# hippylib/hippyflow

Measured on AMD Instinct MI355X. Metric: randomized-SVD throughput (GDoF*rank/s), higher is better.
Workload: dtype f64

## Files before the change

hippyflow_amd/csrc/hfmi_gemm.hip:

```cpp
#include "hfmi_gemm_common.h"

#ifdef HFMI_TN_NT
#define TN_LOAD_A(p) __builtin_nontemporal_load(p)
#else
#define TN_LOAD_A(p) (*(p))
#endif
struct TnTail {
  int nrb, nsplit;
  int64_t chunk;
  double* out;
  int64_t si, sj, sps;
};

template <int MT, int NT, bool TR, int WAVES, int R4>
__global__ __launch_bounds__(WAVES * 64, (WAVES == 8 || MT * NT <= 20) ? 2 : 1) void k_tsgemm_tn(const double* __restrict__ A, int64_t lda, int m,
                                                                    const double* B , int64_t ldb, int k,
                                                                    int64_t Npad, int64_t chunk, int nrb, int nsplit,
                                                                    double* __restrict__ out, int64_t si, int64_t sj,
                                                                    int64_t sps, int direct, int probe_arg, TnTail tail) {
#ifdef HFMI_TN_PROBE
  const int probe = probe_arg;
#else
  constexpr int probe = 0;
  (void)probe_arg;
#endif
  extern __shared__ __attribute__((aligned(16))) char smem[];
  constexpr int BK = TN_BK;
  constexpr int COLS = NT * 16;
  constexpr int LDB = BK + 2;
  constexpr int BUFD = COLS * LDB;
  constexpr int CSH = 4;
  constexpr int NTF = R4 > 0 ? NT - 1 : NT;
  constexpr int NR4 = R4 > 0 ? R4 : 1;
  constexpr int NTHR = WAVES * 64;
  constexpr int CH = COLS * (BK / 2);
  constexpr int NQ = (CH + NTHR - 1) / NTHR;
  constexpr int EST = MT * NTF * 8 + MT * R4 * 2 + NTF * 4 + R4 * 4 + 16 * MT + NQ * 6;
  constexpr int AH = (EST <= ((WAVES == 8 || MT * NT <= 20) ? 218 : 470)) ? 2 : 1;
  double* lds = reinterpret_cast<double*>(smem);
  const int tid = threadIdx.x, lane = tid & 63, wave = tid >> 6;
  const int r16 = lane & 15, kk = lane >> 4;

  const int nfull = nrb * nsplit;
  const bool in_tail = (int)blockIdx.x >= nfull;
  const int logical = in_tail ? xcd_remap((int)blockIdx.x - nfull, tail.nrb * tail.nsplit) : xcd_remap(blockIdx.x, nfull);
  const int sp = in_tail ? logical / tail.nrb : logical / nrb;
  const int rb = in_tail ? nrb + logical % tail.nrb : logical % nrb;
  if (in_tail) {
    chunk = tail.chunk;
    out = tail.out;
    si = tail.si;
    sj = tail.sj;
    sps = tail.sps;
    direct = 0;
  }
  const int row_off = in_tail ? nrb * (16 * MT * WAVES) : 0;
  const int64_t t_begin = (int64_t)sp * chunk;
  int64_t t_end = t_begin + chunk;
  if (t_end > Npad) t_end = Npad;
  const int nstages = (int)((t_end - t_begin) / BK);
  const int64_t t_last = t_end - 8 * AH;
  const int rowbase = rb * (16 * MT * WAVES) + wave * (16 * MT);

  const double* a_ptr[MT];
#pragma unroll
  for (int mt = 0; mt < MT; ++mt) {
    int row = rowbase + mt * 16 + r16;
    if (row > m - 1) row = m - 1;
    a_ptr[mt] = A + (int64_t)row * lda + kk * 2 * AH;
  }
  const double* b_ptr[NQ];
#pragma unroll
  for (int qd = 0; qd < NQ; ++qd) {
    int c = tid + NTHR * qd;
    if (c > CH - 1) c = CH - 1;
    int col = c >> CSH;
    if (col > k - 1) col = k - 1;
    b_ptr[qd] = B + (int64_t)col * ldb + (c & ((1 << CSH) - 1)) * 2;
  }

  constexpr int NTA = NTF > 0 ? NTF : 1;
  d4 acc[MT][NTA];
  double acc4[MT][NR4];
#pragma unroll
  for (int mt = 0; mt < MT; ++mt) {
#pragma unroll
    for (int nt = 0; nt < NTA; ++nt) acc[mt][nt] = d4{0.0, 0.0, 0.0, 0.0};
#pragma unroll
    for (int q = 0; q < NR4; ++q) acc4[mt][q] = 0.0;
  }

  d2 breg[NQ];
  auto stage_load = [&](int64_t ts) {
#pragma unroll
    for (int qd = 0; qd < NQ; ++qd) breg[qd] = *reinterpret_cast<const d2*>(b_ptr[qd] + ts);
  };
  auto stage_store = [&](double* L) {
#pragma unroll
    for (int qd = 0; qd < NQ; ++qd) {
      const int c = tid + NTHR * qd;
      const int col = c >> CSH, q = c & ((1 << CSH) - 1);
      const int off = col * LDB + q * 2;
      if (CH % NTHR == 0 || c < CH) *reinterpret_cast<d2*>(L + off) = breg[qd];
    }
  };
  auto load_a = [&](d2(&dst)[AH][MT], int64_t t) {
    if (t > t_last) t = t_last;
    if (probe & 1) t = t_begin;
#pragma unroll
    for (int mt = 0; mt < MT; ++mt)
#pragma unroll
      for (int h = 0; h < AH; ++h) dst[h][mt] = TN_LOAD_A(reinterpret_cast<const d2*>(a_ptr[mt] + t + 2 * h));
  };
  d2 bf[NTA];
  auto koff = [&](int it) { return (it / AH) * (8 * AH) + kk * (2 * AH) + (it % AH) * 2; };
  auto ldsb1 = [&](const double* L, int it, int nt) {
    bf[nt] = *reinterpret_cast<const d2*>(L + (nt * 16 + r16) * LDB + koff(it));
  };
  auto mma = [&](const d2(&a)[MT], const double* L, int it, bool refill) {
    d2 bg[NR4];
    if constexpr (R4 > 0) {
#pragma unroll
      for (int q = 0; q < R4; ++q)
        bg[q] = *reinterpret_cast<const d2*>(L + (NTF * 16 + 4 * q + (lane & 3)) * LDB + koff(it));
    }
#pragma unroll
    for (int nt = 0; nt < NTF; ++nt) {
#pragma unroll
      for (int mt = 0; mt < MT; ++mt)
        acc[mt][nt] = TR ? MFMA_F64(bf[nt].x, a[mt].x, acc[mt][nt]) : MFMA_F64(a[mt].x, bf[nt].x, acc[mt][nt]);
#pragma unroll
      for (int mt = 0; mt < MT; ++mt)
        acc[mt][nt] = TR ? MFMA_F64(bf[nt].y, a[mt].y, acc[mt][nt]) : MFMA_F64(a[mt].y, bf[nt].y, acc[mt][nt]);
      if (refill) ldsb1(L, it + 1, nt);
      __builtin_amdgcn_sched_barrier(0);
    }
    if constexpr (R4 > 0) {
#pragma unroll
      for (int mt = 0; mt < MT; ++mt)
#pragma unroll
        for (int q = 0; q < R4; ++q) acc4[mt][q] = MFMA_F64_4(a[mt].x, bg[q].x, acc4[mt][q]);
#pragma unroll
      for (int mt = 0; mt < MT; ++mt)
#pragma unroll
        for (int q = 0; q < R4; ++q) acc4[mt][q] = MFMA_F64_4(a[mt].y, bg[q].y, acc4[mt][q]);
    }
    __builtin_amdgcn_sched_barrier(0);
  };

  if (nstages > 0) {
    stage_load(t_begin);
    stage_store(lds);
    __syncthreads();
  }
  {
    constexpr int NIT = BK / (8 * AH), NH = BK / 8;
    d2 a[2][AH][MT];
    load_a(a[0], t_begin);
    for (int s = 0; s < nstages; ++s) {
      const int64_t ts = t_begin + (int64_t)s * BK;
      const bool has_next = s + 1 < nstages;
      stage_load(has_next ? ts + BK : ts);
      asm volatile("" ::: "memory");
      const double* L = lds + (s & 1) * BUFD;
#pragma unroll
      for (int nt = 0; nt < NTF; ++nt) ldsb1(L, 0, nt);
#pragma unroll
      for (int it = 0; it < NIT; ++it) {
        load_a(a[(it + 1) & 1], ts + 8 * AH * (it + 1));
#pragma unroll
        for (int h = 0; h < AH; ++h) mma(a[it & 1][h], L, it * AH + h, it * AH + h + 1 < NH);
      }
      if (!(probe & 2)) {
      if (has_next) stage_store(lds + ((s + 1) & 1) * BUFD);
      __syncthreads();
      }
    }
  }

  double* P = out + (int64_t)sp * sps;
#pragma unroll
  for (int mt = 0; mt < MT; ++mt)
#pragma unroll
    for (int nt = 0; nt < NTF; ++nt)
#pragma unroll
      for (int r = 0; r < 4; ++r) {
        const int i = TR ? rowbase + mt * 16 + r16 : rowbase + mt * 16 + kk + 4 * r;
        const int j = TR ? nt * 16 + kk + 4 * r : nt * 16 + r16;
        if (!direct || (i < m && j < k)) P[(int64_t)(i - row_off) * si + (int64_t)j * sj] = acc[mt][nt][r];
      }
  if constexpr (R4 > 0) {
    const int i4 = lane >> 4, g4 = (lane >> 2) & 3, j4 = lane & 3;
#pragma unroll
    for (int mt = 0; mt < MT; ++mt)
#pragma unroll
      for (int q = 0; q < R4; ++q) {
        const int i = rowbase + mt * 16 + 4 * g4 + i4;
        const int j = NTF * 16 + 4 * q + j4;
        if (!direct || (i < m && j < k)) P[(int64_t)(i - row_off) * si + (int64_t)j * sj] = acc4[mt][q];
      }
  }
}

template <int RY>
__global__ __launch_bounds__(64 * RY) void k_reduce_partials(const double* __restrict__ part, int nsplit, int64_t pstride,
                                                             int inner_ld, int tr, int m, int k, double scale, double beta,
                                                             double* __restrict__ C, int64_t rs, int64_t cs) {
  __shared__ double sh[RY][64];
  const int tx = threadIdx.x, ty = threadIdx.y;
  const int fast = blockIdx.x * 64 + tx;
  const int fastn = tr ? m : k, slown = tr ? k : m;
  for (int slow = blockIdx.y; slow < slown; slow += gridDim.y) {
    double s0 = 0.0, s1 = 0.0, s2 = 0.0, s3 = 0.0;
    if (fast < fastn) {
      const double* p = part + (int64_t)slow * inner_ld + fast;
      int sp = ty;
      for (; sp + 3 * RY < nsplit; sp += 4 * RY) {
        s0 += p[(int64_t)sp * pstride];
        s1 += p[(int64_t)(sp + RY) * pstride];
        s2 += p[(int64_t)(sp + 2 * RY) * pstride];
        s3 += p[(int64_t)(sp + 3 * RY) * pstride];
      }
      for (; sp < nsplit; sp += RY) s0 += p[(int64_t)sp * pstride];
    }
    sh[ty][tx] = (s0 + s1) + (s2 + s3);
    __syncthreads();
    if (ty == 0 && fast < fastn) {
      double s = 0.0;
#pragma unroll
      for (int y = 0; y < RY; ++y) s += sh[y][tx];
      const int i = tr ? fast : slow, j = tr ? slow : fast;
      double* out = C + (int64_t)i * rs + (int64_t)j * cs;
      *out = (beta != 0.0) ? scale * s + beta * (*out) : scale * s;
    }
    __syncthreads();
  }
}

template <int RY>
__global__ __launch_bounds__(64 * RY) void k_reduce_flat(const double* __restrict__ part, int nsplit, int64_t pstride,
                                                         int64_t total, int kpad, int k, double scale, double beta,
                                                         double* __restrict__ C) {
  __shared__ double sh[RY][64];
  const int tx = threadIdx.x, ty = threadIdx.y;
  const int64_t idx = (int64_t)blockIdx.x * 64 + tx;
  double s0 = 0.0, s1 = 0.0, s2 = 0.0, s3 = 0.0;
  if (idx < total) {
    const double* p = part + idx;
    int sp = ty;
    for (; sp + 3 * RY < nsplit; sp += 4 * RY) {
      s0 += p[(int64_t)sp * pstride];
      s1 += p[(int64_t)(sp + RY) * pstride];
      s2 += p[(int64_t)(sp + 2 * RY) * pstride];
      s3 += p[(int64_t)(sp + 3 * RY) * pstride];
    }
    for (; sp < nsplit; sp += RY) s0 += p[(int64_t)sp * pstride];
  }
  sh[ty][tx] = (s0 + s1) + (s2 + s3);
  __syncthreads();
  if (ty == 0 && idx < total) {
    double s = 0.0;
#pragma unroll
    for (int y = 0; y < RY; ++y) s += sh[y][tx];
    const bool real = (int)(idx % kpad) < k;
    C[idx] = real ? ((beta != 0.0) ? scale * s + beta * C[idx] : scale * s) : 0.0;
  }
}

__global__ __launch_bounds__(256) void k_reduce_vec(const double* __restrict__ part, int nsplit, int64_t pstride, int64_t prow,
                                                    int64_t rowlen, int nrows, int64_t kpad, int kreal, double scale, double beta,
                                                    double* __restrict__ C, int64_t crow) {
  const int64_t f = ((int64_t)blockIdx.x * 256 + threadIdx.x) * 2;
  if (f >= rowlen) return;
  for (int row = blockIdx.y; row < nrows; row += gridDim.y) {
    const double* p = part + (int64_t)row * prow + f;
    d2 s0 = d2{0.0, 0.0}, s1 = s0, s2 = s0, s3 = s0;
    int sp = 0;
    for (; sp + 3 < nsplit; sp += 4) {
      s0 += *reinterpret_cast<const d2*>(p + (int64_t)sp * pstride);
      s1 += *reinterpret_cast<const d2*>(p + (int64_t)(sp + 1) * pstride);
      s2 += *reinterpret_cast<const d2*>(p + (int64_t)(sp + 2) * pstride);
      s3 += *reinterpret_cast<const d2*>(p + (int64_t)(sp + 3) * pstride);
    }
    for (; sp < nsplit; ++sp) s0 += *reinterpret_cast<const d2*>(p + (int64_t)sp * pstride);
    d2 v = ((s0 + s1) + (s2 + s3)) * scale;
    double* out = C + (int64_t)row * crow + f;
    if (beta != 0.0) v += beta * *reinterpret_cast<const d2*>(out);
    if (kreal < kpad) {
      if ((int)(f % kpad) >= kreal) v.x = 0.0;
      if ((int)((f + 1) % kpad) >= kreal) v.y = 0.0;
    }
    *reinterpret_cast<d2*>(out) = v;
  }
}

int launch_reduce_partials(hfmi_ctx* ctx, const double* part, const reduce_call& c, double scale, double beta, double* C, int64_t rs,
                           int64_t cs) {
  const reduce_plan p = reduce_plan_make(c, rs, cs, (((uintptr_t)part | (uintptr_t)C) & 15) == 0);
  const dim3 grid(p.gx, p.gy);
  switch (p.route) {
    case HFMI_REDUCE_VEC_LONG:
    case HFMI_REDUCE_VEC_ROWS:
      hipLaunchKernelGGL(k_reduce_vec, grid, dim3(256), 0, ctx->stream, part, p.nsplit, c.pstride, (int64_t)c.inner_ld, p.rowlen, p.nrows,
                         p.kpad, p.kreal, scale, beta, C, p.crow);
      break;
    case HFMI_REDUCE_FLAT:
      hipLaunchKernelGGL(p.ry == 4 ? k_reduce_flat<4> : k_reduce_flat<16>, grid, dim3(64, p.ry), 0, ctx->stream, part, p.nsplit, c.pstride,
                         p.rowlen, c.inner_ld, p.k, scale, beta, C);
      break;
    default:
      hipLaunchKernelGGL(p.ry == 4 ? k_reduce_partials<4> : k_reduce_partials<16>, grid, dim3(64, p.ry), 0, ctx->stream, part, p.nsplit,
                         c.pstride, c.inner_ld, p.tr, p.m, p.k, scale, beta, C, rs, cs);
  }
  HIP_TRY(hipGetLastError());
  reduce_plan_words(p, plan_slot(ctx));
  return HFMI_OK;
}

typedef void (*tn_kernel_t)(const double*, int64_t, int, const double*, int64_t, int, int64_t, int64_t, int, int, double*, int64_t, int64_t,
                            int64_t, int, int, TnTail);
template <int MT, int NT, int WAVES>
static tn_kernel_t tn_kernel_r4(bool tr, int r4) {
#define TN_R4(R) \
  case R:        \
    return tr ? k_tsgemm_tn<MT, NT, true, WAVES, R> : k_tsgemm_tn<MT, NT, false, WAVES, R>;
  if constexpr (WAVES == 8) {
    switch (r4) { TN_R4(1) TN_R4(2) TN_R4(3) }
  }
  switch (0) { TN_R4(0) }
#undef TN_R4
  return nullptr;
}
template <int NT, int WAVES>
static tn_kernel_t tn_kernel_mt(int mt, bool tr, int r4) {
#define TN_CASE(M) \
  case M:          \
    if constexpr (M * NT <= tn_mt_limit(WAVES)) return tn_kernel_r4<M, NT, WAVES>(tr, r4); \
    break;
  switch (mt) { HFMI_TN_MT_CASES(TN_CASE) }
#undef TN_CASE
  return nullptr;
}
static tn_kernel_t tn_kernel(const tn_plan& p) {
#define TN_NT(NTV) \
  case NTV:        \
    return p.waves == 8 ? tn_kernel_mt<NTV, 8>(p.mt, p.tr, p.r4) : tn_kernel_mt<NTV, 4>(p.mt, p.tr, 0);
  switch (p.nt) { HFMI_TN_NT_CASES(TN_NT) }
#undef TN_NT
  return nullptr;
}

static int tn_panel(hfmi_ctx* ctx, const double* A, int64_t lda, int m, const double* B, int64_t ldb, int k,
                    int64_t N, double scale, double beta, double* C, int64_t rs, int64_t cs, int nsplit_req) {
  const tsgemm_knobs& kn = tsgemm_knobs_ref();
  const tn_plan p = tn_plan_make(m, k, N, scale, beta, rs, cs, C == A || C == B, nsplit_req, kn, ctx->num_cus);
  if (lda % 32 != 0 || ldb % 32 != 0 || lda < p.Npad || ldb < p.Npad)
    HFMI_FAIL(HFMI_ERR_INVALID, "tsgemm_tn: leading dimensions must be multiples of 32 and >= round_up(N,32)");
  const tn_kernel_t kern = p.has_instance ? tn_kernel(p) : nullptr;
  if (!kern) HFMI_FAIL(HFMI_ERR_INVALID, "tsgemm_tn: no instance for MT=%d NT=%d WAVES=%d", p.mt, p.nt, p.waves);
  void* partv = nullptr;
  HFMI_TRY(ctx_ws(ctx, WS_PART, p.ws_bytes, &partv));
  double* part = (double*)partv;
  HIP_TRY(hipFuncSetAttribute((const void*)kern, hipFuncAttributeMaxDynamicSharedMemorySize, (int)p.shmem));
  const int64_t psi = p.tr ? 1 : p.kpad;
  const TnTail tail = {p.tail_nrb, p.tail_nsplit, p.tail_chunk, p.tail_nrb ? part + p.tail_off : nullptr, psi, p.tr ? p.tail_mpad : 1,
                       (int64_t)p.tail_mpad * p.kpad};
  const int pidx = prof_start(ctx, 0, m, k, N);
  hipLaunchKernelGGL(kern, dim3(p.grid), dim3(p.waves * 64), p.shmem, ctx->stream, A, lda, m, B, ldb, k, p.Npad, p.chunk, p.nrb, p.nsplit,
                     p.direct ? C : part, p.direct ? rs : psi, p.direct ? cs : (int64_t)(p.tr ? p.mpad : 1), (int64_t)p.mpad * p.kpad,
                     p.direct ? 1 : 0, kn.probe, tail);
  HIP_TRY(hipGetLastError());
  tn_plan_words(p, plan_slot(ctx));
  prof_stop(ctx, pidx);
  for (int i = 0; i < p.nred; ++i)
    HFMI_TRY(launch_reduce_partials(ctx, part + p.red[i].part_off, p.red[i], scale, beta, C + p.red[i].c_off, rs, cs));
  return HFMI_OK;
}

int launch_tsgemm_tn(hfmi_ctx* ctx, const double* A, int64_t lda, int m, const double* B, int64_t ldb, int k,
                     int64_t N, double scale, double beta, double* C, int64_t rs, int64_t cs, int nsplit_req) {
  if (m <= 0 || k <= 0 || N <= 0) return HFMI_OK;
  if (tsgemm_knobs_ref().ss && ss_applicable(m, k, A == B && lda == ldb && m == k))
    return launch_tsgemm_ss(ctx, A, lda, m, B, ldb, k, N, scale, beta, C, rs, cs, nsplit_req);
  for (int k0 = 0; k0 < k; k0 += 256) {
    const int kp = (k - k0 < 256) ? (k - k0) : 256;
    HFMI_TRY(tn_panel(ctx, A, lda, m, B + (int64_t)k0 * ldb, ldb, kp, N, scale, beta, C + (int64_t)k0 * cs, rs, cs,
                      nsplit_req));
  }
  return HFMI_OK;
}
```

hippyflow_amd/csrc/hfmi_tsgemm_plan.h:

```cpp
#pragma once
#include <stdint.h>
#include <stdlib.h>
#include <string.h>

#include <initializer_list>

#include "hfmi.h"

struct tsgemm_knobs {
  int waves = 8;
  int rem4 = 1;
  int probe = 0;
  int tn_mt = 0;
  int tn_hybrid = 1;
  int ss = 1;
  int ss_percu = 2;
  int ss_blocked = 1;
  int nn_waves = 0;
  int nn_tt = 0;
  int nn_hybrid = 1;
  int nn_res = 1;
  int nn_res_tt = 0;
  int nn_upper = 1;
  int nn_halve_last = 0;
  int env_halve_last = -1;
  bool env_upper_off = false;
};
inline tsgemm_knobs& tsgemm_knobs_ref() {
  static tsgemm_knobs kn = [] {
    tsgemm_knobs k;
    const char* w = getenv("HFMI_GEMM_WAVES");
    k.waves = (w && atoi(w) == 4) ? 4 : (w && atoi(w) == 44) ? 44 : 8;
    const char* h = getenv("HFMI_NN_HALVE_LAST");
    k.env_halve_last = h ? atoi(h) : -1;
    const char* u = getenv("HFMI_NN_UPPER");
    k.env_upper_off = u && atoi(u) == 0;
    return k;
  }();
  return kn;
}
inline bool tsgemm_knob_set(const char* key, int v) {
  tsgemm_knobs& kn = tsgemm_knobs_ref();
  auto put = [&](const char* name, int& field, bool ok) {
    if (strcmp(key, name) != 0 || !ok) return false;
    field = v;
    return true;
  };
  const bool flag = v == 0 || v == 1;
  return put("waves", kn.waves, v == 4 || v == 8 || v == 44) || put("rem4", kn.rem4, flag) || put("probe", kn.probe, true) ||
         put("tn_mt", kn.tn_mt, v >= 0 && v <= 8) || put("tn_hybrid", kn.tn_hybrid, flag) || put("ss", kn.ss, flag) ||
         put("ss_percu", kn.ss_percu, v >= 1 && v <= 4) || put("ss_blocked", kn.ss_blocked, v >= 0 && v <= 2) ||
         put("nn_waves", kn.nn_waves, v == 0 || v == 4 || v == 8) || put("nn_tt", kn.nn_tt, v >= 0 && v <= 3) ||
         put("nn_hybrid", kn.nn_hybrid, flag) || put("nn_res", kn.nn_res, flag) || put("nn_res_tt", kn.nn_res_tt, v >= 0 && v <= 2) ||
         put("nn_upper", kn.nn_upper, flag) || put("nn_halve_last", kn.nn_halve_last, flag);
}

#define HFMI_TN_MT_MAX_W4 0, 8, 8, 8, 8, 6, 5, 4, 4, 3, 3, 2, 2, 2, 2, 2, 2
#define HFMI_TN_MT_MAX_W8 0, 5, 5, 5, 4, 3, 3, 2, 2, 2, 1, 1, 1, 1, 1, 1, 1
#define HFMI_TN_MT_CASES(X) X(1) X(2) X(3) X(4) X(5) X(6) X(8)
#define HFMI_TN_NT_CASES(X) X(1) X(2) X(3) X(4) X(5) X(6) X(7) X(8) X(9) X(10) X(11) X(12) X(13) X(14) X(15) X(16)
constexpr int tn_mt_limit(int waves) { return waves == 8 ? 20 : 32; }
#define HFMI_NN_CASES(X)                                                                                                  \
  X(1, 8, 8) X(2, 8, 8) X(3, 8, 5) X(4, 8, 4) X(5, 6, 3) X(6, 5, 2) X(7, 4, 2) X(8, 4, 2) X(9, 3, 2) X(10, 3, 1) X(11, 2, 1) \
  X(12, 2, 1) X(13, 2, 1) X(14, 2, 1) X(15, 2, 1) X(16, 2, 1)
#define HFMI_NN_RES_CASES(X) X(1, 4) X(2, 4) X(3, 4) X(4, 4) X(5, 3) X(6, 2) X(7, 2) X(8, 2) X(9, 2) X(10, 1)
constexpr int nn_tt_lower(int tt, int by) { return tt > by ? tt - by : 1; }
constexpr int64_t NN_RES_MIN_N = 4096;
constexpr size_t NN_RES_LDS_BYTES = 160 * 1024;
#define HFMI_SS_CASES(X)                                                                                                   \
  X(1, 1) X(1, 2) X(1, 3) X(1, 4) X(1, 5) X(2, 2) X(2, 3) X(2, 4) X(2, 5) X(2, 6) X(3, 5) X(3, 6) X(4, 5) X(4, 6) X(4, 7) X(5, 6) \
  X(5, 7) X(6, 7) X(7, 7) X(7, 8) X(8, 8) X(9, 9) X(10, 9) X(11, 9)                                                        \
  X(3, 3) X(4, 4) X(5, 4) X(6, 5) X(7, 5)
#define HFMI_SSB_CASES(X)                                                                                                  \
  X(2, 5) X(3, 5) X(4, 5) X(5, 5) X(2, 6) X(3, 6) X(4, 6) X(5, 6) X(6, 6) X(2, 9) X(3, 9) X(4, 9) X(5, 9) X(6, 9) X(7, 9) X(8, 9) \
  X(9, 9)

constexpr int TN_BK = 32;
constexpr int NN_KC = 32;
constexpr int SS_BK = 32;

inline int tn_mt_max(int nt, int waves) {
  static const int t4[17] = {HFMI_TN_MT_MAX_W4}, t8[17] = {HFMI_TN_MT_MAX_W8};
  return waves == 4 ? t4[nt] : t8[nt];
}
inline bool tn_has_instance(int mt, int nt, int waves) {
  if (nt < 1 || nt > 16 || mt * nt > tn_mt_limit(waves)) return false;
#define X(M) if (mt == M) return true;
  HFMI_TN_MT_CASES(X)
#undef X
  return false;
}
inline bool nn_case(int nt, int* tt4, int* tt8) {
#define X(NTV, TT4, TT8) if (nt == NTV) { *tt4 = TT4; *tt8 = TT8; return true; }
  HFMI_NN_CASES(X)
#undef X
  return false;
}
inline int nn_res_case(int nt) {
#define X(NTV, TTV) if (nt == NTV) return TTV;
  HFMI_NN_RES_CASES(X)
#undef X
  return 0;
}
inline bool ss_has_instance(int tpw, int nq) {
#define X(T, Q) if (tpw == T && nq == Q) return true;
  HFMI_SS_CASES(X)
#undef X
  return false;
}
inline bool ssb_has_instance(int rt, int ct) {
#define X(R, Cc) if (rt == R && ct == Cc) return true;
  HFMI_SSB_CASES(X)
#undef X
  return false;
}
constexpr int ss_pf(int tpw, int nq) { return (tpw <= 4 && nq <= 6) ? 2 : 1; }

inline int64_t plan_round_up(int64_t x, int64_t m) { return (x + m - 1) / m * m; }
inline int plan_cus(int num_cus) { return num_cus > 0 ? num_cus : 256; }
inline int plan_r4(int cols, int nt, int rem4) {
  const int rem = cols - (nt - 1) * 16;
  return (rem4 && rem <= 12) ? (rem + 3) / 4 : 0;
}
inline void plan_words(int* w, int kind, std::initializer_list<int> fields) {
  int i = 0;
  w[i++] = kind;
  for (int v : fields)
    if (i < HFMI_PLAN_WORDS) w[i++] = v;
  while (i < HFMI_PLAN_WORDS) w[i++] = 0;
}

struct reduce_call {
  int nsplit;
  int64_t pstride;
  int inner_ld;
  bool tr;
  int m, k;
  int64_t part_off, c_off;
};
struct reduce_plan {
  int route, ry;
  int nsplit, tr, m, k;
  unsigned gx, gy;
  int64_t rowlen, kpad, crow;
  int nrows, kreal;
};
inline reduce_plan reduce_plan_make(const reduce_call& c, int64_t rs, int64_t cs, bool ptrs_aligned) {
  reduce_plan p = {};
  const int m = c.m, k = c.k, inner_ld = c.inner_ld;
  const bool tr = c.tr;
  p.nsplit = c.nsplit;
  p.m = m;
  p.k = k;
  const int fastn = tr ? m : k, slown = tr ? k : m;
  const int64_t cfast = tr ? rs : cs, crow = tr ? cs : rs;
  const bool aligned = ptrs_aligned && c.pstride % 2 == 0 && inner_ld % 2 == 0 && crow % 2 == 0;
  if (cfast == 1 && aligned && (int64_t)fastn * slown >= 65536) {
    const bool long_row = !tr && rs == inner_ld;
    if (long_row) {
      p.rowlen = (int64_t)m * inner_ld;
      p.nrows = 1;
      p.kpad = inner_ld;
      p.kreal = k;
    } else {
      p.rowlen = fastn & ~1;
      p.nrows = slown;
    }
    if (p.rowlen == fastn || long_row) {
      p.route = long_row ? HFMI_REDUCE_VEC_LONG : HFMI_REDUCE_VEC_ROWS;
      p.tr = tr ? 1 : 0;
      p.crow = crow;
      p.gx = (unsigned)((p.rowlen / 2 + 255) / 256);
      p.gy = (unsigned)(p.nrows < 32768 ? p.nrows : 32768);
      return p;
    }
  }
  p.ry = c.nsplit <= 32 ? 4 : 16;
  if (!tr && cs == 1 && rs == inner_ld && (int64_t)m * inner_ld >= 65536) {
    p.route = HFMI_REDUCE_FLAT;
    p.rowlen = (int64_t)m * inner_ld;
    p.gx = (unsigned)((p.rowlen + 63) / 64);
    p.gy = 1;
    return p;
  }
  p.route = HFMI_REDUCE_PARTIALS;
  p.tr = tr ? 1 : 0;
  p.gx = (unsigned)((fastn + 63) / 64);
  p.gy = (unsigned)(slown < 32768 ? slown : 32768);
  return p;
}
inline void reduce_plan_words(const reduce_plan& p, int* w) {
  plan_words(w, HFMI_PLAN_REDUCE, {p.route, p.ry, p.nsplit, p.tr, p.m, p.k});
}

struct tn_plan {
  bool has_instance;
  int mt, nt, waves, tr, r4;
  int kpad;
  int64_t Npad;
  size_t shmem;
  int nrb, nsplit, mpad;
  int64_t chunk;
  bool direct;
  int tail_nrb, tail_nsplit, tail_mpad;
  int64_t tail_chunk, tail_off;
  int grid;
  size_t ws_bytes;
  int nred;
  reduce_call red[2];
};
inline tn_plan tn_plan_make(int m, int k, int64_t N, double scale, double beta, int64_t rs, int64_t cs, bool aliased, int nsplit_req,
                            const tsgemm_knobs& kn, int num_cus) {
  tn_plan p = {};
  const int nt = (k + 15) / 16;
  const int kpad = nt * 16;
  const int64_t Npad = plan_round_up(N, TN_BK);
  const bool tr = (rs == 1 && cs != 1);
  const int wcfg = (nt > 11) ? 4 : kn.waves;
  const bool small4 = wcfg == 44;
  const int waves = small4 ? 4 : wcfg;
  const int row_tiles = (m + 15) / 16;
  int mt = nt <= 16 ? tn_mt_max(nt, small4 ? 8 : waves) : 1;
  const int need = (row_tiles + waves - 1) / waves;
  if (need < mt) mt = need;
  if (kn.tn_mt > 0 && kn.tn_mt < mt) mt = kn.tn_mt;
  if (mt == 7) mt = 6;
  if (mt < 1) mt = 1;
  const int rows_per_block = 16 * waves * mt;
  const int nrb = (m + rows_per_block - 1) / rows_per_block;
  const int mpad = nrb * rows_per_block;
  const int cus = plan_cus(num_cus) * (small4 ? 2 : 1);
  const int64_t stages = Npad / TN_BK;
  int nsplit = nsplit_req;
  if (nsplit <= 0) {
    int best = 1;
    double best_cost = 1e300;
    for (int ns = 1; ns <= 128; ++ns) {
      if (ns > 1 && stages / ns < 16) break;
      const int64_t blocks = (int64_t)nrb * ns;
      const int64_t rounds = (blocks + cus - 1) / cus;
      const double eff = (double)blocks / (double)(rounds * cus);
      const double part_ratio = 2.0 * ns * (double)mpad * kpad / ((double)N * (m + k));
      const double cost = 1.0 / eff + part_ratio;
      if (cost < best_cost - 1e-12) {
        best_cost = cost;
        best = ns;
      }
    }
    nsplit = best;
  }
  const bool can_direct = (scale == 1.0 && beta == 0.0 && !aliased);
  int ns_full = 0, nrb_full = 0, ns_tail = 0;
  if (nsplit_req <= 0 && kn.tn_hybrid) {
    const double ideal = (double)nrb / cus;
    const double part_unit = 2.0 * (double)rows_per_block * kpad / ((double)N * (m + k));
    double uniform_cost;
    {
      const int64_t blocks = (int64_t)nrb * nsplit;
      const int64_t rounds = (blocks + cus - 1) / cus;
      uniform_cost = (double)(rounds * cus) / (double)blocks + part_unit * nsplit * nrb;
    }
    double best_cost = uniform_cost;
    static const int cand[] = {1, 2, 3, 4, 6, 8};
    for (int ci = 0; ci < 6; ++ci) {
      const int nsf = cand[ci];
      if (nsf > 1 && stages / nsf < 16) break;
      const int64_t R = ((int64_t)nrb * nsf) / cus;
      if (R < 1 || (R * cus) % nsf != 0) continue;
      const int nf = (int)(R * cus / nsf);
      const int nt_blocks = nrb - nf;
      if (nt_blocks <= 0) continue;
      int nst = cus / nt_blocks;
      if (nst > stages / 16) nst = (int)(stages / 16);
      if (nst > 128) nst = 128;
      if (nst < 1) nst = 1;
      const int64_t tail_rounds = ((int64_t)nt_blocks * nst + cus - 1) / cus;
      const double time = (double)R / nsf + (double)tail_rounds / nst;
      const double parts = part_unit * ((nsf == 1 && can_direct ? 0.0 : (double)nsf * nf) + (double)nst * nt_blocks);
      const double cost = time / ideal + parts;
      if (cost < best_cost - 1e-9) {
        best_cost = cost;
        ns_full = nsf;
        nrb_full = nf;
        ns_tail = nst;
      }
    }
  }
  p.has_instance = tn_has_instance(mt, nt, waves);
  p.mt = mt;
  p.nt = nt;
  p.waves = waves;
  p.tr = tr ? 1 : 0;
  p.r4 = waves == 8 ? plan_r4(k, nt, kn.rem4) : 0;
  p.kpad = kpad;
  p.Npad = Npad;
  p.shmem = (size_t)2 * nt * 16 * (TN_BK + 2) * sizeof(double);
  if (ns_full > 0) {
    const int nrb_t = nrb - nrb_full;
    p.nrb = nrb_full;
    p.mpad = nrb_full * rows_per_block;
    p.chunk = plan_round_up((Npad + ns_full - 1) / ns_full, TN_BK);
    p.nsplit = (int)((Npad + p.chunk - 1) / p.chunk);
    p.tail_nrb = nrb_t;
    p.tail_mpad = nrb_t * rows_per_block;
    p.tail_chunk = plan_round_up((Npad + ns_tail - 1) / ns_tail, TN_BK);
    p.tail_nsplit = (int)((Npad + p.tail_chunk - 1) / p.tail_chunk);
    p.direct = p.nsplit == 1 && can_direct;
    p.tail_off = p.direct ? 0 : (int64_t)p.nsplit * p.mpad * kpad;
    p.ws_bytes = ((size_t)p.tail_off + (size_t)p.tail_nsplit * p.tail_mpad * kpad) * sizeof(double);
    if (!p.direct) p.red[p.nred++] = {p.nsplit, (int64_t)p.mpad * kpad, tr ? p.mpad : kpad, tr, p.mpad, k, 0, 0};
    p.red[p.nred++] = {p.tail_nsplit, (int64_t)p.tail_mpad * kpad, tr ? p.tail_mpad : kpad, tr, m - p.mpad, k, p.tail_off, (int64_t)p.mpad * rs};
  } else {
    p.nrb = nrb;
    p.mpad = mpad;
    p.chunk = plan_round_up((Npad + nsplit - 1) / nsplit, TN_BK);
    if (p.chunk < TN_BK) p.chunk = TN_BK;
    p.nsplit = (int)((Npad + p.chunk - 1) / p.chunk);
    if (p.nsplit < 1) p.nsplit = 1;
    p.direct = p.nsplit == 1 && can_direct;
    p.ws_bytes = (size_t)p.nsplit * mpad * kpad * sizeof(double);
    if (!p.direct) p.red[p.nred++] = {p.nsplit, (int64_t)mpad * kpad, tr ? mpad : kpad, tr, m, k, 0, 0};
  }
  p.grid = p.nrb * p.nsplit + p.tail_nrb * p.tail_nsplit;
  return p;
}
inline void tn_plan_words(const tn_plan& p, int* w) {
  plan_words(w, HFMI_PLAN_TN, {p.mt, p.nt, p.waves, p.tr, p.r4, p.grid, p.nrb, p.nsplit, p.direct ? 1 : 0, p.tail_nrb, p.tail_nsplit});
}

struct nn_launch {
  bool half;
  int grid, tail_tiles, msplit, full_tiles, full_base, tail_base;
  bool reduce;
  int64_t hook_row0, hook_rows;
  int rec_tt, rec_tail;
};
constexpr int NN_MAX_PANELS = 8;
struct nn_plan {
  bool has_instance;
  bool res;
  int tt, nt, waves, r4, upper;
  size_t shmem;
  int tile_rows, ntiles, grid;
  int msplit, mchunk, full_tiles, tail_tiles;
  int64_t ldo, pstride;
  size_t ws_bytes;
  int64_t reduce_row0;
  unsigned reduce_gx;
  bool hooked, halved;
  int nlaunch;
  nn_launch launch[NN_MAX_PANELS + 2];
};
inline double nn_cost(int num_cus, int tile_rows, int m, int r, int64_t N, double rate_factor, int* msplit_out) {
  const int cus = plan_cus(num_cus);
  const int64_t ntiles = (N + tile_rows - 1) / tile_rows;
  const int stages = (m + NN_KC - 1) / NN_KC;
  const double flops = 2.0 * (double)ntiles * tile_rows * (double)m * (double)(((r + 15) / 16) * 16);
  const double rate = 60e12 * rate_factor, hbm = 4.0e12;
  int best = 1;
  double best_t = 1e300;
  for (int ns = 1; ns <= 64; ++ns) {
    if (ns > 1 && stages / ns < 8) break;
    const int64_t blocks = ntiles * ns;
    const int64_t rounds = (blocks + cus - 1) / cus;
    const double eff = (double)blocks / (double)(rounds * cus);
    const double t = flops / (eff * rate) + (ns > 1 ? (ns + 1.0) * (double)N * r * 8.0 / hbm + 3e-6 : 0.0);
    if (t < best_t - 1e-12) {
      best_t = t;
      best = ns;
    }
  }
  *msplit_out = best;
  return best_t;
}
inline void nn_plan_stream(nn_plan& p, int m, int r, int64_t N, int msplit, bool tail_split, int hook_panels, const tsgemm_knobs& kn,
                           int num_cus) {
  const int cus = plan_cus(num_cus);
  const int tile_rows = 16 * p.tt * p.waves;
  const int ntiles = (int)((N + tile_rows - 1) / tile_rows);
  const int sld = p.nt * 16 + ((p.nt % 2 == 0) ? 16 : 0);
  p.shmem = (size_t)2 * NN_KC * sld * sizeof(double);
  p.r4 = plan_r4(r, p.nt, kn.rem4);
  int full_tiles = 0;
  if ((msplit > 1 || tail_split) && ntiles >= cus && kn.nn_hybrid) {
    full_tiles = ntiles / cus * cus;
    const int tail = ntiles - full_tiles;
    if (tail == 0) {
      msplit = 1;
    } else {
      const int stages = (m + NN_KC - 1) / NN_KC;
      int ms = cus / tail;
      if (ms < 2) {
        double best = 1.0;
        ms = 1;
        for (int c = 2; c <= 8; ++c) {
          const double cost = (double)((tail * c + cus - 1) / cus) / c + 0.01 * c;
          if (cost < best - 1e-9) {
            best = cost;
            ms = c;
          }
        }
      }
      if (ms > stages / 4) ms = stages / 4;
      if (ms < 1) ms = 1;
      msplit = ms;
      if (msplit == 1) full_tiles = 0;
    }
  }
  const int mchunk = (int)plan_round_up((m + msplit - 1) / msplit, NN_KC);
  msplit = (m + mchunk - 1) / mchunk;
  if (msplit > 1) {
    p.ldo = plan_round_up(N, 32);
    p.pstride = p.ldo * r;
    p.ws_bytes = (size_t)msplit * p.pstride * sizeof(double);
  } else {
    full_tiles = 0;
  }
  const int tail_tiles = ntiles - full_tiles;
  p.tile_rows = tile_rows, p.ntiles = ntiles, p.msplit = msplit, p.mchunk = mchunk;
  p.full_tiles = full_tiles, p.tail_tiles = tail_tiles, p.grid = full_tiles + tail_tiles * msplit;
  p.reduce_row0 = (int64_t)full_tiles * tile_rows;
  int64_t gx = ((N - p.reduce_row0 + 1) / 2 + 255) / 256;
  if (gx > 2048) gx = 2048;
  if (gx < 1) gx = 1;
  p.reduce_gx = (unsigned)gx;
  auto whole = [&](bool half, int cnt, int first, int64_t row0, int64_t rows) {
    p.launch[p.nlaunch++] = {half, cnt, 1, 1, cnt, first, 0, false, row0, rows, half ? p.tt / 2 : p.tt, 0};
  };
  auto split = [&](int cnt, int first, int tl, bool reduce, int64_t row0, int64_t rows) {
    p.launch[p.nlaunch++] = {false, cnt + tl * msplit, tl > 0 ? tl : 1, msplit, cnt, first, full_tiles, reduce, row0, rows, p.tt, tl};
  };
  const int whole_cnt = msplit > 1 ? full_tiles : ntiles;
  const int rounds = whole_cnt / cus;
  if (hook_panels <= 0 || rounds < 2) {
    split(full_tiles, 0, tail_tiles, msplit > 1, 0, 0);
    return;
  }
  if (hook_panels > NN_MAX_PANELS) hook_panels = NN_MAX_PANELS;
  const int panels = rounds < hook_panels ? rounds : hook_panels;
  const bool on = kn.env_halve_last >= 0 ? kn.env_halve_last != 0 : kn.nn_halve_last != 0;
  p.hooked = true;
  p.halved = on && p.tt % 2 == 0 && panels == rounds && panels + 1 <= hook_panels;
  int base = 0;
  for (int q = 0; q < panels; ++q) {
    const bool last = q == panels - 1;
    const int cnt = last ? whole_cnt - base : (rounds / panels + (q < rounds % panels ? 1 : 0)) * cus;
    const int tl = (last && msplit > 1) ? tail_tiles : 0;
    const int64_t row0 = (int64_t)base * tile_rows, row1 = last ? N : (int64_t)(base + cnt) * tile_rows;
    if (last && p.halved) {
      const int cnt_a = cnt / 2, cnt_b = cnt - cnt_a;
      const int64_t mid = (int64_t)(base + cnt_a) * tile_rows;
      whole(true, 2 * cnt_a, 2 * base, row0, mid - row0);
      whole(true, 2 * cnt_b, 2 * (base + cnt_a), tl > 0 ? 0 : mid, tl > 0 ? 0 : N - mid);
      if (tl > 0) split(0, base, tl, true, mid, N - mid);
    } else if (msplit > 1) {
      split(cnt, base, tl, last, row0, row1 - row0);
    } else {
      whole(false, cnt, base, row0, row1 - row0);
    }
    base += cnt;
  }
}
inline nn_plan nn_plan_make(int m, int r, int64_t N, bool upper_hint, int hook_panels, const tsgemm_knobs& kn, int num_cus) {
  nn_plan p = {};
  const int cus = plan_cus(num_cus);
  const int nt = (r + 15) / 16;
  p.nt = nt;
  p.has_instance = true;
  const int ttv = (kn.nn_res && N >= NN_RES_MIN_N) ? nn_res_case(nt) : 0;
  if (ttv > 0) {
    const int sld = nt * 16 + ((nt % 2 == 0) ? 16 : 0);
    const size_t shmem = (size_t)((m + 3) & ~3) * sld * sizeof(double);
    if (shmem <= NN_RES_LDS_BYTES) {
      auto units = [&](int tt) {
        const int64_t tiles = (N + 128 * tt - 1) / (128 * tt);
        return (double)((tiles + cus - 1) / cus) * tt;
      };
      const int tl = nn_tt_lower(ttv, 1);
      const bool lower = kn.nn_res_tt == 2 || (kn.nn_res_tt == 0 && tl != ttv && units(tl) * 1.05 < units(ttv));
      p.res = true;
      p.tt = lower ? tl : ttv;
      p.waves = 8;
      p.r4 = plan_r4(r, nt, kn.rem4);
      p.upper = (upper_hint && kn.nn_upper && !kn.env_upper_off) ? 1 : 0;
      p.shmem = shmem;
      p.tile_rows = 16 * p.tt * 8;
      p.ntiles = (int)((N + p.tile_rows - 1) / p.tile_rows);
      p.grid = p.ntiles < cus ? p.ntiles : cus;
      p.msplit = 1;
      p.full_tiles = p.ntiles;
      return p;
    }
  }
  int tt4 = 0, tt8 = 0;
  if (!nn_case(nt, &tt4, &tt8)) {
    p.has_instance = false;
    return p;
  }
  p.waves = kn.nn_waves ? kn.nn_waves : (nt >= 7 ? 8 : 4);
  int ms = 1;
  bool tail_split = false;
  if (p.waves == 8) {
    p.tt = tt8;
    nn_cost(num_cus, 128 * tt8, m, r, N, 1.0, &ms);
  } else {
    const int t1 = nn_tt_lower(tt4, 1), t2 = nn_tt_lower(tt4, 2);
    int ms0 = 1, ms1 = 1, ms2 = 1;
    const double c0 = nn_cost(num_cus, 64 * tt4, m, r, N, 1.0, &ms0);
    const double c1 = (t1 != tt4) ? nn_cost(num_cus, 64 * t1, m, r, N, 0.98, &ms1) : 1e300;
    const double c2 = (t2 != t1) ? nn_cost(num_cus, 64 * t2, m, r, N, 0.96, &ms2) : 1e300;
    if (kn.nn_hybrid && kn.nn_tt == 0 && (N + 64 * tt4 - 1) / (64 * tt4) >= cus && m >= 16 * NN_KC) p.tt = tt4, ms = 1, tail_split = true;
    else if (kn.nn_tt == 1) p.tt = tt4, ms = ms0;
    else if (kn.nn_tt == 2) p.tt = t1, ms = ms1;
    else if (kn.nn_tt == 3) p.tt = t2, ms = ms2;
    else if (c0 <= c1 && c0 <= c2) p.tt = tt4, ms = ms0;
    else if (c1 <= c2) p.tt = t1, ms = ms1;
    else p.tt = t2, ms = ms2;
  }
  nn_plan_stream(p, m, r, N, ms, tail_split, hook_panels, kn, num_cus);
  return p;
}
inline void nn_res_plan_words(const nn_plan& p, int* w) {
  plan_words(w, HFMI_PLAN_NN_RES, {p.tt, p.nt, 8, p.r4, p.upper, 1, p.ntiles, 0, p.grid});
}
inline void nn_launch_words(const nn_plan& p, const nn_launch& l, int* w) {
  plan_words(w, HFMI_PLAN_NN, {l.rec_tt, p.nt, p.waves, p.r4, 0, l.msplit, l.full_tiles, l.rec_tail, l.grid});
}

inline bool ss_applicable(int m, int k, bool same) {
  const int rt = (m + 15) / 16, ct = (k + 15) / 16;
  if (rt < 1 || ct < 1 || rt > 10 || ct > 10) return false;
  const int ctot = same ? rt * 16 : (rt + ct) * 16;
  return ctot <= 288;
}
struct ss_plan {
  bool has_instance;
  bool same, swap, blocked, pipe;
  int rt, ct;
  int tpw, nq, pf;
  size_t shmem;
  int per_cu, nsplit;
  int64_t Npad, chunk;
  size_t ws_bytes;
  reduce_call red;
};
inline ss_plan ss_plan_make(int m, int k, int64_t N, bool same, int nsplit_req, const tsgemm_knobs& kn, int num_cus) {
  ss_plan p = {};
  const int rt = (m + 15) / 16, ct = (k + 15) / 16;
  const int ctot = same ? rt * 16 : (rt + ct) * 16;
  p.Npad = plan_round_up(N, SS_BK);
  p.same = same;
  p.swap = !same && rt > ct;
  p.rt = p.swap ? ct : rt;
  p.ct = p.swap ? rt : ct;
  p.blocked = !same && kn.ss_blocked && ssb_has_instance(p.rt, p.ct);
  p.tpw = ((same ? rt * (rt + 1) / 2 : rt * ct) + 7) / 8;
  p.nq = (ctot + 31) / 32;
  p.pf = ss_pf(p.tpw, p.nq);
  p.has_instance = p.blocked || ss_has_instance(p.tpw, p.nq);
  p.pipe = p.blocked && kn.ss_blocked != 2 && p.rt * p.ct <= 56;
  const size_t stage_bytes = (size_t)p.nq * 32 * SS_BK * sizeof(double);
  p.shmem = (p.pf == 2 && !p.blocked) ? stage_bytes : 2 * stage_bytes + (size_t)p.nq * 32 * sizeof(double*);
  int per_cu = (int)((160 * 1024) / p.shmem);
  const int reg_cap = (p.tpw <= 4 && !p.blocked) ? kn.ss_percu : 1;
  if (per_cu > reg_cap) per_cu = reg_cap;
  if (per_cu < 1) per_cu = 1;
  p.per_cu = per_cu;
  const int64_t stages = p.Npad / SS_BK;
  int nsplit = nsplit_req > 0 ? nsplit_req : plan_cus(num_cus) * per_cu;
  if (nsplit > stages / 2) nsplit = (int)(stages / 2);
  if (nsplit < 1) nsplit = 1;
  p.chunk = plan_round_up((p.Npad + nsplit - 1) / nsplit, SS_BK);
  p.nsplit = (int)((p.Npad + p.chunk - 1) / p.chunk);
  const int mpad = rt * 16, kpad = ct * 16;
  p.ws_bytes = (size_t)p.nsplit * mpad * kpad * sizeof(double);
  const bool sw = p.blocked && p.swap;
  p.red = {p.nsplit, (int64_t)mpad * kpad, sw ? mpad : kpad, sw, m, k, 0, 0};
  return p;
}
inline void ss_plan_words(const ss_plan& p, int* w) {
  if (p.blocked) plan_words(w, HFMI_PLAN_SSB, {p.rt, p.ct, p.nq, p.pipe ? 1 : 0, p.swap ? 1 : 0, 0, p.nsplit});
  else plan_words(w, HFMI_PLAN_SS, {p.tpw, p.nq, p.pf, 0, p.same ? 1 : 0, p.nsplit});
}
```

Baseline: 0.1628.

## Add auto TN shape selection and lean pointer mode to cut register pressure

In high-register-estimate configurations, the TN tall-skinny GEMM kernel now keeps a single base pointer for A and for B and derives the other row and column addresses from scalar strides, clamped to the last valid address. This is meant to reduce VGPR pressure. The commit also adds an auto shape selector (8-wave, taller 8-wave, or 4-wave with remainder-4 columns) and enables r4 instances for 4-wave kernels, which increases the number of instantiated variants. The auto-case table is empty, so by default the selector resolves to the 8-wave shape, matching the previous behaviour.

```diff
diff --git a/hippyflow_amd/csrc/hfmi_gemm.hip b/hippyflow_amd/csrc/hfmi_gemm.hip
--- a/hippyflow_amd/csrc/hfmi_gemm.hip
+++ b/hippyflow_amd/csrc/hfmi_gemm.hip
@@ -37,6 +37,8 @@
   constexpr int NQ = (CH + NTHR - 1) / NTHR;
   constexpr int EST = MT * NTF * 8 + MT * R4 * 2 + NTF * 4 + R4 * 4 + 16 * MT + NQ * 6;
   constexpr int AH = (EST <= ((WAVES == 8 || MT * NT <= 20) ? 218 : 470)) ? 2 : 1;
+  constexpr bool LEAN = EST > 256 && (WAVES == 8 || MT * NT <= 20);
+  constexpr int NAP = LEAN ? 1 : MT, NBP = LEAN ? 1 : NQ;
   double* lds = reinterpret_cast<double*>(smem);
   const int tid = threadIdx.x, lane = tid & 63, wave = tid >> 6;
   const int r16 = lane & 15, kk = lane >> 4;
@@ -62,22 +64,25 @@
   const int64_t t_last = t_end - 8 * AH;
   const int rowbase = rb * (16 * MT * WAVES) + wave * (16 * MT);
 
-  const double* a_ptr[MT];
-#pragma unroll
-  for (int mt = 0; mt < MT; ++mt) {
+  const double* a_ptr[NAP];
+#pragma unroll
+  for (int mt = 0; mt < NAP; ++mt) {
     int row = rowbase + mt * 16 + r16;
     if (row > m - 1) row = m - 1;
     a_ptr[mt] = A + (int64_t)row * lda + kk * 2 * AH;
   }
-  const double* b_ptr[NQ];
-#pragma unroll
-  for (int qd = 0; qd < NQ; ++qd) {
+  const double* b_ptr[NBP];
+#pragma unroll
+  for (int qd = 0; qd < NBP; ++qd) {
     int c = tid + NTHR * qd;
     if (c > CH - 1) c = CH - 1;
     int col = c >> CSH;
     if (col > k - 1) col = k - 1;
     b_ptr[qd] = B + (int64_t)col * ldb + (c & ((1 << CSH) - 1)) * 2;
   }
+  const int64_t a_step = 16 * lda, b_step = (int64_t)(NTHR >> CSH) * ldb;
+  const double* const a_cap = A + (int64_t)(m - 1) * lda + 3 * 2 * AH;
+  const double* const b_cap = B + (int64_t)(k - 1) * ldb + 2 * ((1 << CSH) - 1);
 
   constexpr int NTA = NTF > 0 ? NTF : 1;
   d4 acc[MT][NTA];
@@ -93,7 +98,18 @@
   d2 breg[NQ];
   auto stage_load = [&](int64_t ts) {
 #pragma unroll
-    for (int qd = 0; qd < NQ; ++qd) breg[qd] = *reinterpret_cast<const d2*>(b_ptr[qd] + ts);
+    for (int qd = 0; qd < NQ; ++qd) {
+      const double* p;
+      if constexpr (LEAN) {
+        int64_t off = qd * b_step + ts;
+        asm("" : "+s"(off));
+        p = b_ptr[0] + off;
+        if (qd > 0 && p > b_cap + ts) p = b_cap + ts;
+      } else {
+        p = b_ptr[qd] + ts;
+      }
+      breg[qd] = *reinterpret_cast<const d2*>(p);
+    }
   };
   auto stage_store = [&](double* L) {
 #pragma unroll
@@ -108,9 +124,19 @@
     if (t > t_last) t = t_last;
     if (probe & 1) t = t_begin;
 #pragma unroll
-    for (int mt = 0; mt < MT; ++mt)
-#pragma unroll
-      for (int h = 0; h < AH; ++h) dst[h][mt] = TN_LOAD_A(reinterpret_cast<const d2*>(a_ptr[mt] + t + 2 * h));
+    for (int mt = 0; mt < MT; ++mt) {
+      const double* p;
+      if constexpr (LEAN) {
+        int64_t off = mt * a_step + t;
+        asm("" : "+s"(off));
+        p = a_ptr[0] + off;
+        if (mt > 0 && p > a_cap + t) p = a_cap + t;
+      } else {
+        p = a_ptr[mt] + t;
+      }
+#pragma unroll
+      for (int h = 0; h < AH; ++h) dst[h][mt] = TN_LOAD_A(reinterpret_cast<const d2*>(p + 2 * h));
+    }
   };
   d2 bf[NTA];
   auto koff = [&](int it) { return (it / AH) * (8 * AH) + kk * (2 * AH) + (it % AH) * 2; };
@@ -324,9 +350,7 @@
 #define TN_R4(R) \
   case R:        \
     return tr ? k_tsgemm_tn<MT, NT, true, WAVES, R> : k_tsgemm_tn<MT, NT, false, WAVES, R>;
-  if constexpr (WAVES == 8) {
-    switch (r4) { TN_R4(1) TN_R4(2) TN_R4(3) }
-  }
+  switch (r4) { TN_R4(1) TN_R4(2) TN_R4(3) }
   switch (0) { TN_R4(0) }
 #undef TN_R4
   return nullptr;
@@ -344,7 +368,7 @@
 static tn_kernel_t tn_kernel(const tn_plan& p) {
 #define TN_NT(NTV) \
   case NTV:        \
-    return p.waves == 8 ? tn_kernel_mt<NTV, 8>(p.mt, p.tr, p.r4) : tn_kernel_mt<NTV, 4>(p.mt, p.tr, 0);
+    return p.waves == 8 ? tn_kernel_mt<NTV, 8>(p.mt, p.tr, p.r4) : tn_kernel_mt<NTV, 4>(p.mt, p.tr, p.r4);
   switch (p.nt) { HFMI_TN_NT_CASES(TN_NT) }
 #undef TN_NT
   return nullptr;
diff --git a/hippyflow_amd/csrc/hfmi_tsgemm_plan.h b/hippyflow_amd/csrc/hfmi_tsgemm_plan.h
--- a/hippyflow_amd/csrc/hfmi_tsgemm_plan.h
+++ b/hippyflow_amd/csrc/hfmi_tsgemm_plan.h
@@ -8,7 +8,8 @@
 #include "hfmi.h"
 
 struct tsgemm_knobs {
-  int waves = 8;
+  int waves = 0;
+  int tn_shape = 0;
   int rem4 = 1;
   int probe = 0;
   int tn_mt = 0;
@@ -30,7 +31,7 @@
   static tsgemm_knobs kn = [] {
     tsgemm_knobs k;
     const char* w = getenv("HFMI_GEMM_WAVES");
-    k.waves = (w && atoi(w) == 4) ? 4 : (w && atoi(w) == 44) ? 44 : 8;
+    k.waves = !w ? 0 : atoi(w) == 4 ? 4 : atoi(w) == 44 ? 44 : atoi(w) == 8 ? 8 : 0;
     const char* h = getenv("HFMI_NN_HALVE_LAST");
     k.env_halve_last = h ? atoi(h) : -1;
     const char* u = getenv("HFMI_NN_UPPER");
@@ -47,7 +48,8 @@
     return true;
   };
   const bool flag = v == 0 || v == 1;
-  return put("waves", kn.waves, v == 4 || v == 8 || v == 44) || put("rem4", kn.rem4, flag) || put("probe", kn.probe, true) ||
+  return put("waves", kn.waves, v == 0 || v == 4 || v == 8 || v == 44) || put("tn_shape", kn.tn_shape, v >= 0 && v <= 4) ||
+         put("rem4", kn.rem4, flag) || put("probe", kn.probe, true) ||
          put("tn_mt", kn.tn_mt, v >= 0 && v <= 8) || put("tn_hybrid", kn.tn_hybrid, flag) || put("ss", kn.ss, flag) ||
          put("ss_percu", kn.ss_percu, v >= 1 && v <= 4) || put("ss_blocked", kn.ss_blocked, v >= 0 && v <= 2) ||
          put("nn_waves", kn.nn_waves, v == 0 || v == 4 || v == 8) || put("nn_tt", kn.nn_tt, v >= 0 && v <= 3) ||
@@ -89,6 +91,26 @@
   HFMI_TN_MT_CASES(X)
 #undef X
   return false;
+}
+enum {
+  TN_SHAPE_W8 = 1,
+  TN_SHAPE_TALL8 = 2,
+  TN_SHAPE_W44R4 = 3,
+  TN_SHAPE_W4R4 = 4,
+};
+#define HFMI_TN_AUTO_CASES(X)
+inline int tn_auto_shape(int nt, int r4, int force) {
+  int s = TN_SHAPE_W8;
+#define X(NTV, R4V, S) if (nt == NTV && r4 == R4V) s = S;
+  HFMI_TN_AUTO_CASES(X)
+#undef X
+  if (force > 0) s = force;
+  if (nt > 11) return TN_SHAPE_W8;
+  if (s == TN_SHAPE_TALL8) {
+    const int mt = tn_mt_max(nt, 8) + 1;
+    if (mt == 7 || !tn_has_instance(mt, nt, 8)) s = TN_SHAPE_W8;
+  }
+  return s;
 }
 inline bool nn_case(int nt, int* tt4, int* tt8) {
 #define X(NTV, TT4, TT8) if (nt == NTV) { *tt4 = TT4; *tt8 = TT8; return true; }
@@ -216,11 +238,19 @@
   const int kpad = nt * 16;
   const int64_t Npad = plan_round_up(N, TN_BK);
   const bool tr = (rs == 1 && cs != 1);
-  const int wcfg = (nt > 11) ? 4 : kn.waves;
+  int wsel = kn.waves;
+  bool taller = false, auto_r4 = false;
+  if (wsel == 0) {
+    const int shape = tn_auto_shape(nt, plan_r4(k, nt, kn.rem4), kn.tn_shape);
+    wsel = shape == TN_SHAPE_W44R4 ? 44 : shape == TN_SHAPE_W4R4 ? 4 : 8;
+    taller = shape == TN_SHAPE_TALL8;
+    auto_r4 = shape == TN_SHAPE_W44R4 || shape == TN_SHAPE_W4R4;
+  }
+  const int wcfg = (nt > 11) ? 4 : wsel;
   const bool small4 = wcfg == 44;
   const int waves = small4 ? 4 : wcfg;
   const int row_tiles = (m + 15) / 16;
-  int mt = nt <= 16 ? tn_mt_max(nt, small4 ? 8 : waves) : 1;
+  int mt = nt <= 16 ? tn_mt_max(nt, small4 ? 8 : waves) + (taller ? 1 : 0) : 1;
   const int need = (row_tiles + waves - 1) / waves;
   if (need < mt) mt = need;
   if (kn.tn_mt > 0 && kn.tn_mt < mt) mt = kn.tn_mt;
@@ -291,7 +321,7 @@
   p.nt = nt;
   p.waves = waves;
   p.tr = tr ? 1 : 0;
-  p.r4 = waves == 8 ? plan_r4(k, nt, kn.rem4) : 0;
+  p.r4 = (waves == 8 || auto_r4) ? plan_r4(k, nt, kn.rem4) : 0;
   p.kpad = kpad;
   p.Npad = Npad;
   p.shmem = (size_t)2 * nt * 16 * (TN_BK + 2) * sizeof(double);
```

New measurement: 0.1633, median of 4. No clear change (+0.4%).
